# MaxWolf-01/sentinel2-landcover-classification

Measured on AMD Instinct MI355X. Metric: Sentinel-2 256x256x13 tiles/sec fwd+bwd, higher is better.
Workload: dtype f32

## Files before the change

__graft_entry__.py:

```python
from __future__ import annotations

import os
import subprocess
import sys
from pathlib import Path

ROOT = Path(__file__).resolve().parent
PKG = ROOT / "sentinel2-landcover-classification_amd"
CSRC = PKG / "csrc"
LIB = PKG / "libs2k.so"
SOURCES = ["s2k_api.hip", "igemm.hip", "igemm_pc.hip", "conv_dma.hip", "conv_q4.hip", "conv_bf16.hip", "wgrad.hip", "wgrad_pc.hip", "wgrad_q4.hip", "wgrad_bf16.hip", "dwconv.hip", "ew.hip", "loss.hip", "vit.hip", "attn.hip", "input.hip", "predict.hip", "flat_stats.hip", "quicklook.hip", "peaks.hip"]


def _stale() -> bool:
    if not LIB.exists():
        return True
    t = LIB.stat().st_mtime
    deps = [CSRC / s for s in SOURCES] + [CSRC / "common.h", CSRC / "wgrad.h", CSRC / "igemm.h", CSRC / "dma.h", ROOT / "include" / "s2k.h", ROOT / "include" / "s2k_ops.h"]
    return any(d.stat().st_mtime > t for d in deps)


def build_tuning(stamps: bool = False, exact_silu: bool = False) -> Path:
    hipcc = os.environ.get("HIPCC", "/opt/rocm/bin/hipcc")
    out = PKG / ("libs2k_exact.so" if exact_silu else ("libs2k_stamps.so" if stamps else "libs2k_tuning.so"))
    cmd = ([hipcc, "--offload-arch=gfx950", "-O3", "-std=c++17", "-fPIC", "-Wno-unused-value", "-DS2K_TUNING"] + (["-DS2K_DMA_STAMPS"] if stamps else [])
           + (["-DS2K_EXACT_SILU"] if exact_silu else []) + ["-shared", "-o", str(out)])
    cmd += [str(CSRC / s) for s in SOURCES]
    r = subprocess.run(cmd, stdout=subprocess.PIPE, stderr=subprocess.STDOUT, text=True)
    if r.returncode != 0:
        raise RuntimeError(f"tuning build failed:\n{r.stdout}")
    return out


def build(force: bool = False) -> None:
    if str(ROOT) not in sys.path:
        sys.path.insert(0, str(ROOT))
    hipcc = os.environ.get("HIPCC", "/opt/rocm/bin/hipcc")
    have_hipcc = Path(hipcc).exists()
    if (force or _stale()) and have_hipcc:
        objs = []
        procs = []
        for s in SOURCES:
            obj = CSRC / (s + ".o")
            objs.append(str(obj))
# ... 104 lines not shown
```

include/s2k_ops.h:

```cpp
#ifndef S2K_OPS_H
#define S2K_OPS_H

#define S2K_N_T 12
#define S2K_N_N 4
#define S2K_N_D 24
#define S2K_N_F 6

#define S2K_BASE_WS 0
#define S2K_BASE_PARAMS 1
#define S2K_BASE_GRADS 2
#define S2K_BASE_BUFS 3
#define S2K_BASE_X 4
#define S2K_BASE_OUT 5
#define S2K_BASE_DOUT 6
#define S2K_BASE_NOISE 7
#define S2K_BASE_WGS 8
#define S2K_BASE_CONST 9
#define S2K_BASE_Y 10
#define S2K_BASE_AUX 11
#define S2K_BASE_WPACK 12
#define S2K_BASE_DX 13
#define S2K_N_BASES 14

#define S2K_PRO_NONE 0
#define S2K_PRO_AFFINE 1
#define S2K_PRO_SILU 2
#define S2K_PRO_RELU 3
#define S2K_PRO_GELU 4
#define S2K_MODE_CONV 0
#define S2K_MODE_CONVT_SCATTER 1
#define S2K_MODE_GATHER2X2 2
#define S2K_FLAG_SIDE 1
#define S2K_FLAG_JOIN 2
#define S2K_FLAG_BF16 4
#define S2K_FLAG_Q4 16
#define S2K_FLAG_DMA 8
#define S2K_FLAG_RES_GELU_GRAD 32
#define S2K_FLAG_SPLIT 64
#define S2K_FLAG_CHAIN 128

#define S2K_OP_MEMSET 1
#define S2K_MEMSET_T_DST 0
#define S2K_MEMSET_N_BYTES 0

#define S2K_OP_AXPY 2
#define S2K_AXPY_T_X 0
#define S2K_AXPY_T_Y 1
#define S2K_AXPY_N_COUNT 0

#define S2K_OP_WEIGHT_PACK 3
#define S2K_WEIGHT_PACK_T_TABLE 0
#define S2K_WEIGHT_PACK_T_SRC 1
#define S2K_WEIGHT_PACK_T_DST 2
#define S2K_WEIGHT_PACK_N_TOTAL 0
#define S2K_WEIGHT_PACK_N_BF16_BASE 1
#define S2K_WEIGHT_PACK_N_Q4_BASE 2
#define S2K_WEIGHT_PACK_N_SPLIT_BASE 3
#define S2K_WEIGHT_PACK_D_N_ENTRIES 0

#define S2K_OP_CONV 4
#define S2K_CONV_T_X1 0
#define S2K_CONV_T_BNV1 1
#define S2K_CONV_T_GATE1 2
#define S2K_CONV_T_X2 3
#define S2K_CONV_T_BNV2 4
#define S2K_CONV_T_WT 5
#define S2K_CONV_T_BIAS 6
#define S2K_CONV_T_Y 7
#define S2K_CONV_T_STATS 8
#define S2K_CONV_T_RES 9
#define S2K_CONV_T_SCRATCH 10
#define S2K_CONV_T_WTB 11
// ... 722 lines not shown
```

sentinel2-landcover-classification_amd/csrc/s2k_api.hip:

```cpp
#include <cstdarg>
#include <cstdio>
#include <cstring>
#include <mutex>
#include <vector>

#include <stdlib.h>

#include "common.h"

namespace s2k {

static thread_local char g_err[512] = "";
thread_local int g_s2k_variant = 0;

void set_error(const char* fmt, ...) {
    va_list ap;
    va_start(ap, fmt);
    vsnprintf(g_err, sizeof(g_err), fmt, ap);
    va_end(ap);
}

int launch_conv(const S2kOp&, const Ctx&);
int launch_wgrad(const S2kOp&, const Ctx&);
int launch_dwconv_fwd(const S2kOp&, const Ctx&);
int launch_dwconv_dgrad(const S2kOp&, const Ctx&);
int launch_dwconv_wgrad(const S2kOp&, const Ctx&);
int launch_axpy(const S2kOp&, const Ctx&);
int launch_weight_pack(const S2kOp&, const Ctx&);
int launch_wgrad_finalize(const S2kOp&, const Ctx&);
int launch_bn_finalize(const S2kOp&, const Ctx&);
int launch_se_pool(const S2kOp&, const Ctx&);
int launch_se_fc(const S2kOp&, const Ctx&);
// ... 11 lines not shown
int launch_chan_ln_bwd(const S2kOp&, const Ctx&);
int launch_act_bwd(const S2kOp&, const Ctx&);
int launch_act_fwd(const S2kOp&, const Ctx&);
int launch_attn_fwd(const S2kOp&, const Ctx&);
int launch_attn_bwd(const S2kOp&, const Ctx&);
int launch_mae_mask_index(const S2kOp&, const Ctx&);
int launch_token_gather(const S2kOp&, const Ctx&);
int launch_token_scatter(const S2kOp&, const Ctx&);
int launch_patchify(const S2kOp&, const Ctx&);
int launch_mae_loss_fwd(const S2kOp&, const Ctx&);
int launch_mae_loss_bwd(const S2kOp&, const Ctx&);
int launch_transpose_cl(const S2kOp&, const Ctx&);
int launch_drop_gate(const S2kOp&, const Ctx&);
int launch_confusion(const S2kOp&, const Ctx&);
int launch_tile_prep(const S2kOp&, const Ctx&);
int launch_se_bn_sums(const S2kOp&, const Ctx&);
int launch_se_bn_combine(const S2kOp&, const Ctx&);
int launch_space_to_depth(const S2kOp&, const Ctx&);
int launch_se_fc_wgrad(const S2kOp&, const Ctx&);
int launch_ids_to_dec_idx(const S2kOp&, const Ctx&);
int launch_upsample_zero(const S2kOp&, const Ctx&);
int launch_im2col(const S2kOp&, const Ctx&);
int launch_tile_label_hist(const S2kOp&, const Ctx&);
int launch_tile_moments(const S2kOp&, const Ctx&);
int launch_window_blend(const S2kOp&, const Ctx&);
int launch_seg_stats(const S2kOp&, const Ctx&);
int launch_seg_hist(const S2kOp&, const Ctx&);
int launch_grad_clip(const S2kOp&, const Ctx&);
int launch_tile_radix_hist(const S2kOp&, const Ctx&);
int launch_tile_rank_pick(const S2kOp&, const Ctx&);
int launch_tile_quicklook(const S2kOp&, const Ctx&);
int launch_class_overlay(const S2kOp&, const Ctx&);
int launch_dw_bwd_chain(const S2kOp*, const Ctx&);
int launch_adam(float*, const float*, float*, float*, int64_t, double, double, double, double, double, int, hipStream_t);
int launch_mfma_selftest(const float*, const float*, float*, hipStream_t);

static int launch_memset(const S2kOp& op, const Ctx& c) {
    const int64_t ref = op.t[S2K_MEMSET_T_DST];
    const int64_t bytes = op.n[S2K_MEMSET_N_BYTES];
    if (ref < 0 || bytes <= 0) { set_error("memset: bad args"); return S2K_EINVAL; }
    const int base = (int)(ref >> 56);
    if (base >= c.n_bases || !c.bases[base]) { set_error("memset: null base %d", base); return S2K_EFAULT; }
    char* dst = static_cast<char*>(c.bases[base]) + (ref & ((1ll << 56) - 1));
    if (hipMemsetAsync(dst, 0, (size_t)bytes, c.stream) != hipSuccess) { set_error("memset: hipMemsetAsync failed"); return S2K_EHIP; }
    return S2K_OK;
}

static const char* const kNames[S2K_N_KINDS + 1] = {
    nullptr,
    "MEMSET", "AXPY", "WEIGHT_PACK", "CONV", "WGRAD", "WGRAD_FINALIZE", "DWCONV_FWD", "DWCONV_DGRAD", "DWCONV_WGRAD",
    "BN_FINALIZE", "SE_POOL", "SE_FC", "SE_FC_BWD", "SE_BWD_REDUCE", "BN_BWD_REDUCE", "BN_BWD_FINALIZE", "BN_BWD_APPLY",
    "BN_RESIDUAL", "CHANNEL_SUM", "LOSS_FWD", "LOSS_BWD", "ARGMAX", "CHAN_LN_FWD", "CHAN_LN_BWD", "ACT_BWD", "ACT_FWD",
    "ATTN_FWD", "ATTN_BWD", "MAE_MASK_INDEX", "IDS_TO_DEC_IDX", "TOKEN_GATHER", "TOKEN_SCATTER", "PATCHIFY", "MAE_LOSS_FWD",
    "MAE_LOSS_BWD", "TRANSPOSE_CL", "CONFUSION", "DROP_GATE", "TILE_PREP", "SE_BN_SUMS", "SE_BN_COMBINE", "SPACE_TO_DEPTH",
    "UPSAMPLE_ZERO", "SE_FC_WGRAD", "IM2COL", "TILE_LABEL_HIST", "TILE_MOMENTS", "WINDOW_BLEND",
    "SEG_STATS", "SEG_HIST", "GRAD_CLIP", "TILE_RADIX_HIST", "TILE_RANK_PICK", "TILE_QUICKLOOK", "CLASS_OVERLAY"};

static int dispatch(const S2kOp& op, const Ctx& c) {
    switch (op.kind) {
        case S2K_OP_MEMSET: return launch_memset(op, c);
        case S2K_OP_AXPY: return launch_axpy(op, c);
        case S2K_OP_WEIGHT_PACK: return launch_weight_pack(op, c);
        case S2K_OP_CONV: return launch_conv(op, c);
        case S2K_OP_WGRAD: return launch_wgrad(op, c);
        case S2K_OP_WGRAD_FINALIZE: return launch_wgrad_finalize(op, c);
        case S2K_OP_DWCONV_FWD: return launch_dwconv_fwd(op, c);
// ... 141 lines not shown
};

static int try_dw_chain(const S2kOp* ops, int i, int end, const Ctx& c, int* rc) {
    if (!(ops[i].flags & S2K_FLAG_CHAIN) || i + 3 >= end) return 0;
    const S2kOp &a1 = ops[i], &wg = ops[i + 1], &dg = ops[i + 2], &a2 = ops[i + 3];
    if (a1.kind != S2K_OP_BN_BWD_APPLY || wg.kind != S2K_OP_DWCONV_WGRAD || dg.kind != S2K_OP_DWCONV_DGRAD || a2.kind != S2K_OP_BN_BWD_APPLY) return 0;
    if ((a1.flags | wg.flags | dg.flags | a2.flags) & (S2K_FLAG_BF16 | S2K_FLAG_SPLIT)) return 0;
    const int64_t dy = a1.t[S2K_BN_BWD_APPLY_T_DY], x = dg.t[S2K_DWCONV_DGRAD_T_XRAW], g = dg.t[S2K_DWCONV_DGRAD_T_G];
    if (dy < 0 || a1.t[S2K_BN_BWD_APPLY_T_GP] != dy || a1.t[S2K_BN_BWD_APPLY_T_COEF] >= 0 || a1.t[S2K_BN_BWD_APPLY_T_PS] < 0 ||
        a1.t[S2K_BN_BWD_APPLY_T_MULBC] < 0 || a1.t[S2K_BN_BWD_APPLY_T_ADDBC] < 0 || a1.d[S2K_BN_BWD_APPLY_D_ACT] != S2K_PRO_SILU ||
        a1.d[S2K_BN_BWD_APPLY_D_EVAL] || a1.d[S2K_BN_BWD_APPLY_D_OUT_BF16] || a1.n[S2K_BN_BWD_APPLY_N_COUNT] <= 0) return 0;
    if (wg.t[S2K_DWCONV_WGRAD_T_DY] != dy || dg.t[S2K_DWCONV_DGRAD_T_DY] != dy || x < 0 || wg.t[S2K_DWCONV_WGRAD_T_X] != x ||
        dg.t[S2K_DWCONV_DGRAD_T_BNV] < 0 || wg.t[S2K_DWCONV_WGRAD_T_BNV] != dg.t[S2K_DWCONV_DGRAD_T_BNV] || g < 0 || g == dy || g == x ||
        dg.t[S2K_DWCONV_DGRAD_T_STATS2] < 0) return 0;
    for (int k = 0; k <= 10; ++k)
        if (wg.d[k] != dg.d[k]) return 0;
    const int B = dg.d[0], C = dg.d[1], H = dg.d[2], W = dg.d[3], K = dg.d[4];
    if (B <= 0 || C <= 0 || H != W || (W != 8 && W != 16) || (K != 3 && K != 5) || dg.d[5] != 1 || dg.d[6] != (K - 1) / 2 || dg.d[7] != (K - 1) / 2 ||
        dg.d[8] != H || dg.d[9] != W || dg.d[10] != S2K_PRO_SILU || dg.d[S2K_DWCONV_DGRAD_D_BETA] != 0) return 0;
    if ((int64_t)B * C * H * W * 4 >= 0x7ffffff0ll) return 0;
    if (a2.t[S2K_BN_BWD_APPLY_T_GP] != g || a2.t[S2K_BN_BWD_APPLY_T_DY] != g || a2.t[S2K_BN_BWD_APPLY_T_Y] != x ||
        a2.t[S2K_BN_BWD_APPLY_T_BNV] != dg.t[S2K_DWCONV_DGRAD_T_BNV] || a2.t[S2K_BN_BWD_APPLY_T_STATS2] != dg.t[S2K_DWCONV_DGRAD_T_STATS2] ||
        a2.t[S2K_BN_BWD_APPLY_T_COEF] >= 0 || a2.t[S2K_BN_BWD_APPLY_T_PS] >= 0 || a2.t[S2K_BN_BWD_APPLY_T_MULBC] >= 0 ||
        a2.t[S2K_BN_BWD_APPLY_T_ADDBC] >= 0 || a2.d[S2K_BN_BWD_APPLY_D_ACT] != S2K_PRO_NONE || a2.d[S2K_BN_BWD_APPLY_D_EVAL] ||
        a2.d[S2K_BN_BWD_APPLY_D_OUT_BF16] || a2.n[S2K_BN_BWD_APPLY_N_COUNT] <= 0) return 0;
    const int HW = H * W;
    if (a1.d[S2K_BN_BWD_APPLY_D_B] != B || a1.d[S2K_BN_BWD_APPLY_D_C] != C || a1.d[S2K_BN_BWD_APPLY_D_HW] != HW ||
        a2.d[S2K_BN_BWD_APPLY_D_B] != B || a2.d[S2K_BN_BWD_APPLY_D_C] != C || a2.d[S2K_BN_BWD_APPLY_D_HW] != HW) return 0;
    g_s2k_variant = 0;
    *rc = check_launch(launch_dw_bwd_chain(&ops[i], c), ops[i], i);
    return 4;
}

int s2k_program_run(const S2kOp* ops, int begin, int end, void* const* bases, int n_bases, void* stream) {
    if (!ops || !bases || begin < 0 || end < begin) { set_error("program_run: bad arguments"); return S2K_EINVAL; }
    hipStream_t main_st = static_cast<hipStream_t>(stream);
    DeviceGuard guard(main_st);
    Ctx c{bases, n_bases, main_st};
    bool any_side = false;
    for (int i = begin; i < end && !any_side; ++i) any_side = (ops[i].flags & S2K_FLAG_SIDE) != 0;
    SideQueue* sq = any_side ? lease_side_queue(guard.dev) : nullptr;
    bool side_busy = false;
    bool main_dirty = true;
    auto join = [&]() {
        if (!side_busy) return;
        (void)hipEventRecord(sq->join, sq->stream);
        (void)hipStreamWaitEvent(main_st, sq->join, 0);
        side_busy = false;
    };
    int rc = S2K_OK;
    for (int i = begin; i < end; ++i) {
        const S2kOp& op = ops[i];
        if ((op.flags & S2K_FLAG_CHAIN) && i + 3 < end) {
            if ((op.flags | ops[i + 1].flags | ops[i + 2].flags | ops[i + 3].flags) & S2K_FLAG_JOIN) join();
            const int used = try_dw_chain(ops, i, end, c, &rc);
            if (used) {
                main_dirty = true;
                if (rc != S2K_OK) break;
                i += used - 1;
                continue;
            }
        }
        if ((op.flags & S2K_FLAG_SIDE) && sq) {
            if (main_dirty) {
                (void)hipEventRecord(sq->fork, main_st);
                (void)hipStreamWaitEvent(sq->stream, sq->fork, 0);
                main_dirty = false;
            }
            Ctx cs{bases, n_bases, sq->stream};
            rc = check_launch(dispatch(op, cs), op, i);
            side_busy = true;
        } else {
            if (op.flags & S2K_FLAG_JOIN) join();
            rc = check_launch(dispatch(op, c), op, i);
            main_dirty = true;
        }
        if (rc != S2K_OK) break;
    }
    join();
    release_side_queue(guard.dev, sq);
    return rc;
}

int s2k_op_launch(const S2kOp* op, void* const* bases, int n_bases, void* stream) {
    if (!op || !bases) { set_error("op_launch: bad arguments"); return S2K_EINVAL; }
    DeviceGuard guard(static_cast<hipStream_t>(stream));
    Ctx c{bases, n_bases, static_cast<hipStream_t>(stream)};
    return check_launch(dispatch(*op, c), *op, 0);
}

static int profile_impl(const S2kOp* ops, int begin, int end, void* const* bases, int n_bases, void* stream, float* ms_by_kind,
                        int* launches_by_kind, float* ms_per_op, int* variant_per_op);

int s2k_program_profile(const S2kOp* ops, int begin, int end, void* const* bases, int n_bases, void* stream, float* ms_by_kind,
                        int* launches_by_kind) {
// ... 3 lines not shown
int s2k_program_profile_ops(const S2kOp* ops, int begin, int end, void* const* bases, int n_bases, void* stream,
                            float* ms_per_op) {
    float ms[S2K_N_KINDS + 1];
    int cnt[S2K_N_KINDS + 1];
    return profile_impl(ops, begin, end, bases, n_bases, stream, ms, cnt, ms_per_op, nullptr);
}

int s2k_program_profile_variants(const S2kOp* ops, int begin, int end, void* const* bases, int n_bases, void* stream,
                                 float* ms_per_op, int* variant_per_op) {
    float ms[S2K_N_KINDS + 1];
    int cnt[S2K_N_KINDS + 1];
    if (!ms_per_op || !variant_per_op) { set_error("program_profile_variants: bad arguments"); return S2K_EINVAL; }
    return profile_impl(ops, begin, end, bases, n_bases, stream, ms, cnt, ms_per_op, variant_per_op);
}

static int profile_impl(const S2kOp* ops, int begin, int end, void* const* bases, int n_bases, void* stream, float* ms_by_kind,
                        int* launches_by_kind, float* ms_per_op, int* variant_per_op) {
    if (!ops || !bases || !ms_by_kind || !launches_by_kind || begin < 0 || end < begin) {
        set_error("program_profile: bad arguments");
        return S2K_EINVAL;
    }
    hipStream_t st = static_cast<hipStream_t>(stream);
    DeviceGuard guard(st);
    Ctx c{bases, n_bases, st};
    const int n = end - begin;
    hipEvent_t* ev = new hipEvent_t[n + 1];
    for (int i = 0; i <= n; ++i) hipEventCreate(&ev[i]);
    int rc = S2K_OK;
    hipEventRecord(ev[0], st);
    int done = 0;
    std::vector<char> fused(n, 0);
    for (int i = 0; i < n; ++i) {
        g_s2k_variant = 0;
        const int used = try_dw_chain(ops, begin + i, end, c, &rc);
        if (!used) rc = check_launch(dispatch(ops[begin + i], c), ops[begin + i], begin + i);
        if (rc != S2K_OK) break;
        for (int k = 0; k < (used ? used : 1); ++k) {
            if (variant_per_op) variant_per_op[i + k] = g_s2k_variant;
            hipEventRecord(ev[i + k + 1], st);
            if (k) fused[i + k] = 1;
        }
        if (used) i += used - 1;
        done = i + 1;
    }
    hipStreamSynchronize(st);
    if (rc == S2K_OK) {
        for (int k = 0; k <= S2K_N_KINDS; ++k) { ms_by_kind[k] = 0.0f; launches_by_kind[k] = 0; }
        for (int i = 0; i < done; ++i) {
            float ms = 0.0f;
            if (!fused[i]) hipEventElapsedTime(&ms, ev[i], ev[i + 1]);
            const int k = ops[begin + i].kind;
            if (ms_per_op) ms_per_op[i] = ms;
            if (k > 0 && k <= S2K_N_KINDS && !fused[i]) { ms_by_kind[k] += ms; launches_by_kind[k] += 1; }
        }
    }
    for (int i = 0; i <= n; ++i) hipEventDestroy(ev[i]);
    delete[] ev;
    return rc;
}

int s2k_adam_step(float* p, const float* g, float* m, float* v, int64_t n, double lr, double beta1, double beta2, double eps,
                  double weight_decay, int step, void* stream) {
    DeviceGuard guard(static_cast<hipStream_t>(stream));
    const int rc = launch_adam(p, g, m, v, n, lr, beta1, beta2, eps, weight_decay, step, static_cast<hipStream_t>(stream));
    if (rc != S2K_OK) return rc;
    const hipError_t e = hipGetLastError();
// ... 15 lines not shown
```

sentinel2-landcover-classification_amd/plan/opdefs.py:

```python
from __future__ import annotations

N_T, N_N, N_D, N_F = 12, 4, 24, 6
OP_BYTES = 8 + 8 * N_T + 8 * N_N + 4 * N_D + 4 * N_F
assert OP_BYTES == 256

BASES = ["WS", "PARAMS", "GRADS", "BUFS", "X", "OUT", "DOUT", "NOISE", "WGS", "CONST", "Y", "AUX", "WPACK", "DX"]
BASE = {n: i for i, n in enumerate(BASES)}

def stats_replicas(C: int) -> int:
    return max(1, min(64, 4096 // max(C, 1)))


PRO_NONE, PRO_AFFINE, PRO_SILU, PRO_RELU, PRO_GELU = 0, 1, 2, 3, 4
ACT_NONE, ACT_SILU, ACT_RELU, ACT_GELU = 0, 2, 3, 4
ACT_MUL = 5
MODE_CONV, MODE_CONVT_SCATTER, MODE_GATHER2X2 = 0, 1, 2
FLAG_SIDE, FLAG_JOIN = 1, 2
FLAG_BF16 = 4
FLAG_Q4 = 16
FLAG_RES_GELU_GRAD = 32
FLAG_SPLIT = 64
FLAG_DMA = 8
FLAG_CHAIN = 128

FOLD_T, FOLD_N, FOLD_D, FOLD_F = ["FSTATS", "FGAMMA", "FBETA", "FRM", "FRV"], ["FCOUNT"], ["FNREP"], ["FEPS", "FMOM"]
FOLD_KINDS = ("DWCONV_FWD", "SE_POOL", "BN_RESIDUAL")

OPS: dict[str, tuple[list[str], list[str], list[str], list[str]]] = {
    "MEMSET": (["DST"], ["BYTES"], [], []),
    "AXPY": (["X", "Y"], ["COUNT"], [], []),
    "WEIGHT_PACK": (["TABLE", "SRC", "DST"], ["TOTAL", "BF16_BASE", "Q4_BASE", "SPLIT_BASE"], ["N_ENTRIES"], []),
    "CONV": (["X1", "BNV1", "GATE1", "X2", "BNV2", "WT", "BIAS", "Y", "STATS", "RES", "SCRATCH", "WTB"], [],
             ["B", "C1", "C2", "H", "W", "M", "KH", "KW", "STRIDE", "PAD_T", "PAD_L", "HO", "WO",
              "PRO1", "PRO2", "MODE", "W_SM", "W_SK", "W_ST", "FLIP", "BETA", "YC", "NREP", "X1_BF16"], []),
    "WGRAD": (["P", "BNVP", "GATEP", "Q", "BNVQ", "GATEQ", "WGS"], [],
              ["B", "M", "C", "CTOT", "H", "W", "KH", "KW", "STRIDE", "PAD_T", "PAD_L", "HO", "WO",
               "PROP", "PROQ", "MODE", "P_BF16"], []),
    "WGRAD_FINALIZE": (["TABLE", "WGS", "GRADS"], ["TOTAL"], ["N_ENTRIES"], []),
    "DWCONV_FWD": (["X", "BNV", "WT", "Y", "STATS"] + FOLD_T, FOLD_N,
                   ["B", "C", "H", "W", "K", "STRIDE", "PAD_T", "PAD_L", "HO", "WO", "PRO", "NREP"] + FOLD_D, FOLD_F),
    "DWCONV_DGRAD": (["DY", "WT", "XRAW", "BNV", "G", "STATS2"], [],
                     ["B", "C", "H", "W", "K", "STRIDE", "PAD_T", "PAD_L", "HO", "WO", "PRO", "BETA", "NREP"], []),
    "DWCONV_WGRAD": (["DY", "X", "BNV", "DW"], [],
                     ["B", "C", "H", "W", "K", "STRIDE", "PAD_T", "PAD_L", "HO", "WO", "PRO"], []),
    "BN_FINALIZE": (["STATS", "GAMMA", "BETA", "RM", "RV", "BNV"], ["COUNT"], ["C", "TRAIN", "NREP"], ["EPS", "MOM"]),
    "SE_POOL": (["Y", "BNV", "POOL"] + FOLD_T, FOLD_N, ["B", "C", "HW", "PRO"] + FOLD_D, FOLD_F),
    "SE_FC": (["POOL", "W1", "B1", "W2", "B2", "HPRE", "GATE"], [], ["B", "C", "CSQ"], []),
    "SE_FC_BWD": (["DGATE", "GATE", "HPRE", "POOL", "W1", "W2", "DW1", "DB1", "DW2", "DB2", "DPOOL", "HS"], [],
                  ["B", "C", "CSQ"], []),
    "SE_BWD_REDUCE": (["G", "Y", "BNV", "DGATE"], [], ["B", "C", "HW", "PRO"], []),
    "BN_BWD_REDUCE": (["G", "Y", "BNV", "MULBC", "ADDBC", "NOISE", "GOUT", "STATS2"], [],
                      ["B", "C", "HW", "ACT", "NREP"], ["KEEP", "ADDSCALE"]),
    "BN_BWD_FINALIZE": (["STATS2", "GAMMA", "BNV", "DGAMMA", "DBETA", "COEF"], ["COUNT"], ["C", "NREP"], []),
    "BN_BWD_APPLY": (["GP", "Y", "BNV", "COEF", "DY", "STATS2", "GAMMA", "DGAMMA", "DBETA", "MULBC", "ADDBC", "PS"], ["COUNT"],
                     ["B", "C", "HW", "NREP", "ACT", "EVAL", "OUT_BF16"], ["ADDSCALE"]),
    "BN_RESIDUAL": (["Y", "BNV", "IDENT", "NOISE", "XOUT"] + FOLD_T, FOLD_N, ["B", "C", "HW"] + FOLD_D, ["KEEP"] + FOLD_F),
# ... 85 lines not shown
```

sentinel2-landcover-classification_amd/plan/unet_plan.py:

```python
from __future__ import annotations

import math
from dataclasses import dataclass, field

from . import opdefs as D
from .program import Arena, Program, TRef

CAT_SIZES = {
    "b0": [592, 296, 152, 80], "b1": [592, 296, 152, 80], "b2": [600, 304, 152, 80],
    "b3": [608, 304, 160, 88], "b4": [624, 312, 160, 88], "b5": [640, 320, 168, 88],
    "b6": [656, 328, 168, 96], "b7": [672, 336, 176, 96],
}


@dataclass
class BlockSpec:
    kernel: int
    stride: int
    cin: int
    cout: int
    expand: int
    se: int
    residual: bool

# ... 717 lines not shown
        if bwd_aux_end > fwd_aux_end:
            pre_ops.append(("MEMSET", dict(DST=TRef(D.BASE["AUX"], fwd_aux_end, (1,), "f32"),
                                           BYTES=bwd_aux_end - fwd_aux_end)))
        p.bwd.ops[0:0] = pre_ops
        segments = _bucket_backward(p, layout, table, bucket_floats)
        side_max = float(tune("S2K_SIDE_MAX_GFLOP", "1e9")) * 1e9
        finalize_on_side = tune("S2K_FINALIZE_SIDE", "1") != "0"
        for kind, f in p.bwd.ops:
            if kind == "WGRAD" and 2.0 * f["M"] * f["C"] * f["KH"] * f["KW"] * f["B"] * f["HO"] * f["WO"] > side_max:
                continue
            if kind in ("WGRAD", "DWCONV_WGRAD", "CHANNEL_SUM", "SE_FC_WGRAD"):
                f["_flags"] = D.FLAG_SIDE
            elif kind == "WGRAD_FINALIZE":
                f["_flags"] = D.FLAG_SIDE if finalize_on_side else D.FLAG_JOIN
        side_stream_hazards(p.bwd)
        n_before = len(p.bwd.ops)
        attach_q4()
        if not bwd_pack_in_fwd:
            pack_op(p.bwd, p.pack_rows["bwd"])
        if len(p.bwd.ops) > n_before:
            segments = [(a + 1 if a else 0, b + 1, lo, hi) for (a, b, lo, hi) in segments]
        bwd = p.bwd
    else:
        attach_q4()
    pack_op(p.fwd, p.pack_rows["fwd"])
    if bwd_pack_in_fwd:
        pack_op(p.fwd, p.pack_rows["bwd"], D.FLAG_SIDE)
    attach_splitk_scratch()
    if getattr(p, "bf16", False):
        mark_bf16(p, bwd)
    if getattr(p, "split", False):
        mark_split(p, bwd)
    mark_dw_chain(p, bwd, segments)
    return segments, bwd


def side_stream_hazards(prog: Program) -> int:
    def ranges(f, names):
        out = []
        for k in names:
            v = f.get(k)
            if isinstance(v, TRef):
                out.append((v.base, v.off, v.off + v.nbytes))
        return out

    pending: list = []
    added = 0
    for kind, f in prog.ops:
        flags = f.get("_flags", 0)
        t_names = D.OPS[kind][0]
        writes = D.WRITES.get(kind, tuple(t_names))
        if flags & D.FLAG_SIDE:
            pending.extend(ranges(f, [k for k in t_names if k not in writes]))
            continue
        if flags & D.FLAG_JOIN:
            pending.clear()
            continue
        if pending:
            for (b, lo, hi) in ranges(f, writes):
                if any(b == pb and lo < phi and plo < hi for (pb, plo, phi) in pending):
                    f["_flags"] = flags | D.FLAG_JOIN
                    pending.clear()
                    added += 1
                    break
    return added

# ... 92 lines not shown
        if tuple(k for k, _ in ops[i:i + 4]) != kinds or seg_end.get(i, 0) < i + 4:
            continue
        a1, wg, dg, a2 = (f for _, f in ops[i:i + 4])
        if any(f.get("_flags", 0) & bad_flags for f in (a1, wg, dg, a2)):
            continue
        dy, x, g, st2 = a1.get("DY"), dg.get("XRAW"), dg.get("G"), dg.get("STATS2")
        if not (same(a1.get("GP"), dy) and same(wg.get("DY"), dy) and same(dg.get("DY"), dy)
                and same(wg.get("X"), x) and same(a2.get("Y"), x) and same(a2.get("GP"), g) and same(a2.get("DY"), g)
                and same(a2.get("STATS2"), st2) and same(wg.get("BNV"), dg.get("BNV")) and same(a2.get("BNV"), dg.get("BNV"))):
            continue
        if not (a1.get("ACT") == D.ACT_SILU and isinstance(a1.get("PS"), TRef) and isinstance(a1.get("MULBC"), TRef)
                and isinstance(a1.get("ADDBC"), TRef) and a1.get("COEF") is None and not a1.get("EVAL") and not a1.get("OUT_BF16")):
            continue
        if not (a2.get("COEF") is None and not a2.get("ACT") and a2.get("PS") is None and a2.get("MULBC") is None
                and a2.get("ADDBC") is None and not a2.get("EVAL") and not a2.get("OUT_BF16")):
            continue
        geo = ("B", "C", "H", "W", "K", "STRIDE", "PAD_T", "PAD_L", "HO", "WO", "PRO")
        K, W = dg["K"], dg["W"]
        if not (all(wg[k] == dg[k] for k in geo) and dg["STRIDE"] == 1 and dg["PRO"] == D.PRO_SILU and not dg.get("BETA")
                and dg["H"] == W and W in (8, 16) and K in (3, 5) and dg["HO"] == W and dg["WO"] == W
                and dg["PAD_T"] == (K - 1) // 2 and dg["PAD_L"] == (K - 1) // 2):
            continue
        if not all(f["B"] == dg["B"] and f["C"] == dg["C"] and f["HW"] == W * W for f in (a1, a2)):
            continue
        dead = [(t.base, t.off, t.off + t.nbytes) for t in (st2,)]
        live = False
        for _k2, f2 in ops[i + 4:]:
            for v in f2.values():
                if isinstance(v, TRef) and any(v.base == b and v.off < hi and lo < v.off + v.nbytes for (b, lo, hi) in dead):
                    live = True
        if live:
            continue
        a1["_flags"] = a1.get("_flags", 0) | D.FLAG_CHAIN
        marked += 1
    return marked


def fold_bn_finalize(prog: Program) -> int:
    if tune("S2K_FOLD_BN", "1") != "1":
        return 0
    ops = prog.ops
    folded = 0
    i = 0
    while i < len(ops):
        kind, f = ops[i]
        if kind != "BN_FINALIZE" or not f.get("TRAIN") or f.get("_flags"):
            i += 1
            continue
        bnv = f["BNV"]
        touched = {t.ref for k in ("BNV", "RM", "RV", "STATS") if isinstance(t := f.get(k), TRef)}
        target = None
        for j in range(i + 1, len(ops)):
            k2, f2 = ops[j]
            refs = {v.ref for v in f2.values() if isinstance(v, TRef)}
            if not (refs & touched):
                continue
            if (k2 in D.FOLD_KINDS and isinstance(f2.get("BNV"), TRef) and f2["BNV"].ref == bnv.ref and f2.get("FSTATS") is None
                    and f2.get("C") == f["C"] and f2.get("PRO", 1) and len(refs & touched) == 1 and not f2.get("_flags")):
                target = j
            break
        if target is None:
            i += 1
            continue
        ops[target][1].update(FSTATS=f["STATS"], FGAMMA=f["GAMMA"], FBETA=f["BETA"], FRM=f["RM"], FRV=f["RV"], FCOUNT=f["COUNT"],
                              FNREP=f["NREP"], FEPS=f["EPS"], FMOM=f["MOM"])
        del ops[i]
# ... 107 lines not shown
```

Before: 999.9.

## Fuse BN backward reduce and apply into paired kernels without materialized gradient

Adds a bn_pair path that detects adjacent BN_BWD_REDUCE/BN_BWD_APPLY ops writing the pre-BN gradient in place. It recomputes that gradient (mul/add/drop-connect/activation grad) inside both the reduce and apply kernels instead of writing it out and reading it back. For small spatial sizes a single per-channel kernel does the reduction and the apply, optionally keeping the loaded data in registers. The aim is to cut memory traffic and one launch per BN backward, at the cost of recomputing the activation gradient and adding planner and runtime matching logic.

Result: no change. 1007 (median of 6 runs) (+0.7%).

```diff
diff --git a/__graft_entry__.py b/__graft_entry__.py
--- a/__graft_entry__.py
+++ b/__graft_entry__.py
@@ -9,7 +9,7 @@
 PKG = ROOT / "sentinel2-landcover-classification_amd"
 CSRC = PKG / "csrc"
 LIB = PKG / "libs2k.so"
-SOURCES = ["s2k_api.hip", "igemm.hip", "igemm_pc.hip", "conv_dma.hip", "conv_q4.hip", "conv_bf16.hip", "wgrad.hip", "wgrad_pc.hip", "wgrad_q4.hip", "wgrad_bf16.hip", "dwconv.hip", "ew.hip", "loss.hip", "vit.hip", "attn.hip", "input.hip", "predict.hip", "flat_stats.hip", "quicklook.hip", "peaks.hip"]
+SOURCES = ["s2k_api.hip", "igemm.hip", "igemm_pc.hip", "conv_dma.hip", "conv_q4.hip", "conv_bf16.hip", "wgrad.hip", "wgrad_pc.hip", "wgrad_q4.hip", "wgrad_bf16.hip", "dwconv.hip", "ew.hip", "bn_pair.hip", "loss.hip", "vit.hip", "attn.hip", "input.hip", "predict.hip", "flat_stats.hip", "quicklook.hip", "peaks.hip"]
 
 
 def _stale() -> bool:
diff --git a/include/s2k_ops.h b/include/s2k_ops.h
--- a/include/s2k_ops.h
+++ b/include/s2k_ops.h
@@ -38,6 +38,7 @@
 #define S2K_FLAG_RES_GELU_GRAD 32
 #define S2K_FLAG_SPLIT 64
 #define S2K_FLAG_CHAIN 128
+#define S2K_FLAG_BN_PAIR 256
 
 #define S2K_OP_MEMSET 1
 #define S2K_MEMSET_T_DST 0
diff --git a/sentinel2-landcover-classification_amd/csrc/bn_pair.hip b/sentinel2-landcover-classification_amd/csrc/bn_pair.hip
--- /dev/null
+++ b/sentinel2-landcover-classification_amd/csrc/bn_pair.hip
@@ -0,0 +1,309 @@
+#include "common.h"
+
+namespace s2k {
+
+namespace {
+
+constexpr int PAIR_CHUNK = 4096;
+constexpr int PAIR_SMALL_HW = 256;
+constexpr int PAIR_SMALL_C = 512;
+
+template <typename T>
+T* ref_ptr(const Ctx& c, int64_t ref) {
+    if (ref < 0) return nullptr;
+    const int base = (int)(ref >> 56);
+    const int64_t off = ref & ((1ll << 56) - 1);
+    if (base >= c.n_bases || c.bases[base] == nullptr) return reinterpret_cast<T*>(1);
+    return reinterpret_cast<T*>(static_cast<char*>(c.bases[base]) + off);
+}
+bool bad(const void* q) { return q == reinterpret_cast<const void*>(1); }
+
+struct PairTask {
+    int64_t plane;
+    int start, count;
+};
+
+__device__ __forceinline__ bool pair_task(int HW, int64_t nplanes, PairTask& t) {
+    const int chunks = (HW + PAIR_CHUNK - 1) / PAIR_CHUNK;
+    const int64_t task = (int64_t)blockIdx.x * 4 + (threadIdx.x >> 6);
+    if (task >= nplanes * chunks) return false;
+    t.plane = (int64_t)((uint32_t)task / (uint32_t)chunks);
+    const int ck = (int)(task - t.plane * chunks);
+    t.start = ck * PAIR_CHUNK;
+    t.count = min(PAIR_CHUNK, HW - t.start);
+    return true;
+}
+
+struct PairArgs {
+    const float *g, *y, *bnv, *mulbc, *addbc, *noise;
+    int C, HW, act;
+    int64_t nplanes;
+    float keep, addscale;
+};
+
+__device__ __forceinline__ void pair_mul_add(const PairArgs& p, int64_t plane, int b, float& mul, float& add) {
+    mul = p.mulbc ? p.mulbc[plane] : 1.0f;
+    if (p.noise) mul *= floorf(p.keep + p.noise[b]) / p.keep;
+    add = p.addbc ? p.addbc[plane] * p.addscale : 0.0f;
+}
+
+__device__ __forceinline__ float pair_gp(float g, float y, float mul, float add, float scale, float shift, int act) {
+    float v = fmaf(g, mul, add);
+    if (act != S2K_PRO_NONE) v *= act_grad(fmaf(y, scale, shift), act);
+    return v;
+}
+
+}
+
+template <bool VEC>
+__global__ void __launch_bounds__(NTHREADS) bn_pair_reduce_kernel(const PairArgs p, double* stats2, int nrep) {
+    PairTask t;
+    if (!pair_task(p.HW, p.nplanes, t)) return;
+    const int lane = threadIdx.x & 63;
+    const int C = p.C;
+    const int c = (int)((uint32_t)t.plane % (uint32_t)C);
+    const int b = (int)((uint32_t)t.plane / (uint32_t)C);
+    const float scale = p.bnv[c], shift = p.bnv[C + c], mean = p.bnv[2 * C + c], invstd = p.bnv[3 * C + c];
+    float mul, add;
+    pair_mul_add(p, t.plane, b, mul, add);
+    const int64_t base = t.plane * p.HW + t.start;
+    const float* g = p.g + base;
+    const float* y = p.y + base;
+    float s1 = 0.0f, s2 = 0.0f;
+    if (VEC) {
+        const int n4 = t.count >> 2;
+        for (int i = lane; i < n4; i += 128) {
+            const int j = min(i + 64, n4 - 1);
+            const bool second = i + 64 < n4;
+            const float4 g0 = reinterpret_cast<const float4*>(g)[i], y0 = reinterpret_cast<const float4*>(y)[i];
+            const float4 g1 = reinterpret_cast<const float4*>(g)[j], y1 = reinterpret_cast<const float4*>(y)[j];
+            const float* gp0 = &g0.x;
+            const float* yp0 = &y0.x;
+            const float* gp1 = &g1.x;
+            const float* yp1 = &y1.x;
+#pragma unroll
+            for (int k = 0; k < 4; ++k) {
+                const float v = pair_gp(gp0[k], yp0[k], mul, add, scale, shift, p.act);
+                s1 += v;
+                s2 = fmaf(v, (yp0[k] - mean) * invstd, s2);
+            }
+#pragma unroll
+            for (int k = 0; k < 4; ++k) {
+                float v = pair_gp(gp1[k], yp1[k], mul, add, scale, shift, p.act);
+                v = second ? v : 0.0f;
+                s1 += v;
+                s2 = fmaf(v, (yp1[k] - mean) * invstd, s2);
+            }
+        }
+    } else {
+        for (int i = lane; i < t.count; i += 64) {
+            const float yy = y[i];
+            const float v = pair_gp(g[i], yy, mul, add, scale, shift, p.act);
+            s1 += v;
+            s2 = fmaf(v, (yy - mean) * invstd, s2);
+        }
+    }
+    s1 = wave_sum(s1);
+    s2 = wave_sum(s2);
+    if (lane == 0) {
+        double* st = stats2 + (int64_t)(blockIdx.x % nrep) * 2 * C;
+        atomic_add_d(st + c, (double)s1);
+        atomic_add_d(st + C + c, (double)s2);
+    }
+}
+
+template <bool VEC>
+__global__ void __launch_bounds__(NTHREADS) bn_pair_apply_kernel(const PairArgs p, float* out, const BnFuse fz) {
+    PairTask t;
+    if (!pair_task(p.HW, p.nplanes, t)) return;
+    const int lane = threadIdx.x & 63;
+    const int C = p.C;
+    const int c = (int)((uint32_t)t.plane % (uint32_t)C);
+    const int b = (int)((uint32_t)t.plane / (uint32_t)C);
+    const int64_t base = t.plane * p.HW + t.start;
+    const float* g = p.g + base;
+    const float* y = p.y + base;
+    float* o = out + base;
+    const int n4 = t.count >> 2;
+    float4 gv0 = make_float4(0, 0, 0, 0), yv0 = make_float4(0, 0, 0, 0);
+    if (VEC && lane < n4) {
+        gv0 = reinterpret_cast<const float4*>(g)[lane];
+        yv0 = reinterpret_cast<const float4*>(y)[lane];
+    }
+    const float scale = p.bnv[c], shift = p.bnv[C + c], mean = p.bnv[2 * C + c], invstd = p.bnv[3 * C + c];
+    float mul, add;
+    pair_mul_add(p, t.plane, b, mul, add);
+    double s1, s2;
+    bn_fuse_sums(fz, C, c, lane, s1, s2);
+    const double aa = (double)fz.gamma[c] * (double)invstd;
+    const float A = (float)aa, Bq = (float)(-aa * s2 * fz.inv_count), Cq = (float)(-aa * s1 * fz.inv_count);
+    const float k0 = A, k1 = Bq * invstd, k2 = Cq - Bq * invstd * mean;
+    if (t.plane < C && t.start == 0 && lane == 0) {
+        fz.dgamma[c] += (float)s2;
+        fz.dbeta[c] += (float)s1;
+    }
+    if (VEC) {
+        for (int i = lane; i < n4; i += 64) {
+            const float4 gv = gv0, yv = yv0;
+            if (i + 64 < n4) {
+                gv0 = reinterpret_cast<const float4*>(g)[i + 64];
+                yv0 = reinterpret_cast<const float4*>(y)[i + 64];
+            }
+            float4 r;
+            r.x = fmaf(k0, pair_gp(gv.x, yv.x, mul, add, scale, shift, p.act), fmaf(k1, yv.x, k2));
+            r.y = fmaf(k0, pair_gp(gv.y, yv.y, mul, add, scale, shift, p.act), fmaf(k1, yv.y, k2));
+            r.z = fmaf(k0, pair_gp(gv.z, yv.z, mul, add, scale, shift, p.act), fmaf(k1, yv.z, k2));
+            r.w = fmaf(k0, pair_gp(gv.w, yv.w, mul, add, scale, shift, p.act), fmaf(k1, yv.w, k2));
+            reinterpret_cast<float4*>(o)[i] = r;
+        }
+    } else {
+        for (int i = lane; i < t.count; i += 64) {
+            const float yy = y[i];
+            o[i] = fmaf(k0, pair_gp(g[i], yy, mul, add, scale, shift, p.act), fmaf(k1, yy, k2));
+        }
+    }
+}
+
+template <int U, bool KEEP>
+__global__ void __launch_bounds__(NTHREADS) bn_pair_small_kernel(const PairArgs p, float* out, const BnFuse fz, int B) {
+    __shared__ double red[8];
+    const int c = blockIdx.x, C = p.C, HW = p.HW;
+    const int n4 = HW >> 2, items = B * n4;
+    const float scale = p.bnv[c], shift = p.bnv[C + c], mean = p.bnv[2 * C + c], invstd = p.bnv[3 * C + c];
+    float4 gv[U], yv[U];
+    float mul[U], add[U];
+    int64_t off[U];
+    double d1 = 0.0, d2 = 0.0;
+    auto load = [&](int q0) {
+#pragma unroll
+        for (int u = 0; u < U; ++u) {
+            const int q = min(q0 + u * NTHREADS, items - 1);
+            const int b = (int)((uint32_t)q / (uint32_t)n4), li = q - b * n4;
+            const int64_t plane = (int64_t)b * C + c;
+            off[u] = plane * HW + 4 * li;
+            gv[u] = *reinterpret_cast<const float4*>(p.g + off[u]);
+            yv[u] = *reinterpret_cast<const float4*>(p.y + off[u]);
+            pair_mul_add(p, plane, b, mul[u], add[u]);
+        }
+    };
+    const int lane = threadIdx.x & 63;
+    const bool aligned = (n4 & (n4 - 1)) == 0;
+    for (int w0 = threadIdx.x - lane; w0 < items; w0 += U * NTHREADS) {
+        const int q0 = w0 + lane;
+        load(q0);
+        float t1 = 0.0f, t2 = 0.0f;
+#pragma unroll
+        for (int u = 0; u < U; ++u) {
+            const bool ok = q0 + u * NTHREADS < items;
+            const float* gp = &gv[u].x;
+            const float* yp = &yv[u].x;
+            float s1 = 0.0f, s2 = 0.0f;
+#pragma unroll
+            for (int k = 0; k < 4; ++k) {
+                const float v = pair_gp(gp[k], yp[k], mul[u], add[u], scale, shift, p.act);
+                s1 += v;
+                s2 = fmaf(v, (yp[k] - mean) * invstd, s2);
+            }
+            s1 = ok ? s1 : 0.0f;
+            s2 = ok ? s2 : 0.0f;
+            if (aligned) {
+                s1 = group_sum(s1, n4);
+                s2 = group_sum(s2, n4);
+                const bool first = (q0 & (n4 - 1)) == 0;
+                d1 += first ? (double)s1 : 0.0;
+                d2 += first ? (double)s2 : 0.0;
+            } else {
+                t1 += s1;
+                t2 += s2;
+            }
+        }
+        d1 += (double)t1;
+        d2 += (double)t2;
+    }
+    d1 = wave_sum_d(d1);
+    d2 = wave_sum_d(d2);
+    if ((threadIdx.x & 63) == 0) { red[threadIdx.x >> 6] = d1; red[4 + (threadIdx.x >> 6)] = d2; }
+    __syncthreads();
+    const double s1 = ((red[0] + red[1]) + red[2]) + red[3], s2 = ((red[4] + red[5]) + red[6]) + red[7];
+    const double aa = (double)fz.gamma[c] * (double)invstd;
+    const float A = (float)aa, Bq = (float)(-aa * s2 * fz.inv_count), Cq = (float)(-aa * s1 * fz.inv_count);
+    const float k0 = A, k1 = Bq * invstd, k2 = Cq - Bq * invstd * mean;
+    if (threadIdx.x == 0) {
+        fz.dgamma[c] += (float)s2;
+        fz.dbeta[c] += (float)s1;
+    }
+    for (int q0 = threadIdx.x; q0 < items; q0 += U * NTHREADS) {
+        if (!KEEP) load(q0);
+#pragma unroll
+        for (int u = 0; u < U; ++u) {
+            if (q0 + u * NTHREADS >= items) break;
+            const float4 g = gv[u], y = yv[u];
+            float4 r;
+            r.x = fmaf(k0, pair_gp(g.x, y.x, mul[u], add[u], scale, shift, p.act), fmaf(k1, y.x, k2));
+            r.y = fmaf(k0, pair_gp(g.y, y.y, mul[u], add[u], scale, shift, p.act), fmaf(k1, y.y, k2));
+            r.z = fmaf(k0, pair_gp(g.z, y.z, mul[u], add[u], scale, shift, p.act), fmaf(k1, y.z, k2));
+            r.w = fmaf(k0, pair_gp(g.w, y.w, mul[u], add[u], scale, shift, p.act), fmaf(k1, y.w, k2));
+            *reinterpret_cast<float4*>(out + off[u]) = r;
+        }
+    }
+}
+
+int launch_bn_pair(const S2kOp* o, const Ctx& c, hipEvent_t mid, int* took) {
+    *took = 0;
+    const S2kOp &r = o[0], &a = o[1];
+    PairArgs p{};
+    p.g = ref_ptr<const float>(c, r.t[S2K_BN_BWD_REDUCE_T_G]);
+    p.y = ref_ptr<const float>(c, r.t[S2K_BN_BWD_REDUCE_T_Y]);
+    p.bnv = ref_ptr<const float>(c, r.t[S2K_BN_BWD_REDUCE_T_BNV]);
+    p.mulbc = ref_ptr<const float>(c, r.t[S2K_BN_BWD_REDUCE_T_MULBC]);
+    p.addbc = ref_ptr<const float>(c, r.t[S2K_BN_BWD_REDUCE_T_ADDBC]);
+    p.noise = ref_ptr<const float>(c, r.t[S2K_BN_BWD_REDUCE_T_NOISE]);
+    float* out = ref_ptr<float>(c, a.t[S2K_BN_BWD_APPLY_T_DY]);
+    double* st2 = ref_ptr<double>(c, r.t[S2K_BN_BWD_REDUCE_T_STATS2]);
+    BnFuse fz{};
+    fz.st2 = st2;
+    fz.gamma = ref_ptr<const float>(c, a.t[S2K_BN_BWD_APPLY_T_GAMMA]);
+    fz.dgamma = ref_ptr<float>(c, a.t[S2K_BN_BWD_APPLY_T_DGAMMA]);
+    fz.dbeta = ref_ptr<float>(c, a.t[S2K_BN_BWD_APPLY_T_DBETA]);
+    const void* ptrs[] = {p.g, p.y, p.bnv, p.mulbc, p.addbc, p.noise, out, st2, fz.gamma, fz.dgamma, fz.dbeta};
+    for (const void* q : ptrs)
+        if (bad(q)) { set_error("bn_pair: tensor references a null base"); return S2K_EFAULT; }
+    const int B = r.d[S2K_BN_BWD_REDUCE_D_B], C = r.d[S2K_BN_BWD_REDUCE_D_C], HW = r.d[S2K_BN_BWD_REDUCE_D_HW];
+    const int64_t count = a.n[S2K_BN_BWD_APPLY_N_COUNT];
+    if (!p.g || !p.y || !p.bnv || !out || !st2 || !fz.gamma || !fz.dgamma || !fz.dbeta || B <= 0 || C <= 0 || HW <= 0 || count <= 0) return S2K_OK;
+    const int64_t nplanes = (int64_t)B * C;
+    const int64_t tasks = nplanes * ((HW + PAIR_CHUNK - 1) / PAIR_CHUNK);
+    if (nplanes * HW * 4 >= 0x7ffffff0ll || tasks >= 0xffffffffll) return S2K_OK;
+    p.C = C; p.HW = HW; p.nplanes = nplanes;
+    p.act = r.d[S2K_BN_BWD_REDUCE_D_ACT];
+    p.keep = r.f[S2K_BN_BWD_REDUCE_F_KEEP];
+    p.addscale = r.f[S2K_BN_BWD_REDUCE_F_ADDSCALE];
+    fz.inv_count = 1.0 / (double)count;
+    fz.nrep = r.d[S2K_BN_BWD_REDUCE_D_NREP] > 0 ? r.d[S2K_BN_BWD_REDUCE_D_NREP] : 1;
+    const int64_t items = (int64_t)B * (HW >> 2);
+    if (HW <= PAIR_SMALL_HW && (HW & 3) == 0 && (items <= 2 * NTHREADS || C >= PAIR_SMALL_C)) {
+        if (items <= 2 * NTHREADS)
+            hipLaunchKernelGGL((bn_pair_small_kernel<2, true>), dim3(C), dim3(NTHREADS), 0, c.stream, p, out, fz, B);
+        else if (items <= 8 * NTHREADS)
+            hipLaunchKernelGGL((bn_pair_small_kernel<8, true>), dim3(C), dim3(NTHREADS), 0, c.stream, p, out, fz, B);
+        else
+            hipLaunchKernelGGL((bn_pair_small_kernel<4, false>), dim3(C), dim3(NTHREADS), 0, c.stream, p, out, fz, B);
+        *took = 2;
+        return S2K_OK;
+    }
+    if (HW <= 64 && (HW & 3) == 0 && B >= 2) return S2K_OK;
+    const unsigned blocks = (unsigned)cdiv64(tasks, 4);
+    if ((HW & 3) == 0) {
+        hipLaunchKernelGGL((bn_pair_reduce_kernel<true>), dim3(blocks), dim3(NTHREADS), 0, c.stream, p, st2, fz.nrep);
+        if (mid) (void)hipEventRecord(mid, c.stream);
+        hipLaunchKernelGGL((bn_pair_apply_kernel<true>), dim3(blocks), dim3(NTHREADS), 0, c.stream, p, out, fz);
+    } else {
+        hipLaunchKernelGGL((bn_pair_reduce_kernel<false>), dim3(blocks), dim3(NTHREADS), 0, c.stream, p, st2, fz.nrep);
+        if (mid) (void)hipEventRecord(mid, c.stream);
+        hipLaunchKernelGGL((bn_pair_apply_kernel<false>), dim3(blocks), dim3(NTHREADS), 0, c.stream, p, out, fz);
+    }
+    *took = 1;
+    return S2K_OK;
+}
+
+}
diff --git a/sentinel2-landcover-classification_amd/csrc/s2k_api.hip b/sentinel2-landcover-classification_amd/csrc/s2k_api.hip
--- a/sentinel2-landcover-classification_amd/csrc/s2k_api.hip
+++ b/sentinel2-landcover-classification_amd/csrc/s2k_api.hip
@@ -1,3 +1,4 @@
+#include <algorithm>
 #include <cstdarg>
 #include <cstdio>
 #include <cstring>
@@ -75,6 +76,7 @@
 int launch_tile_quicklook(const S2kOp&, const Ctx&);
 int launch_class_overlay(const S2kOp&, const Ctx&);
 int launch_dw_bwd_chain(const S2kOp*, const Ctx&);
+int launch_bn_pair(const S2kOp*, const Ctx&, hipEvent_t, int*);
 int launch_adam(float*, const float*, float*, float*, int64_t, double, double, double, double, double, int, hipStream_t);
 int launch_mfma_selftest(const float*, const float*, float*, hipStream_t);
 
@@ -282,6 +284,30 @@
     return 4;
 }
 
+static int try_bn_pair(const S2kOp* ops, int i, int end, const Ctx& c, int* rc, hipEvent_t mid = nullptr) {
+    if (!(ops[i].flags & S2K_FLAG_BN_PAIR) || i + 1 >= end) return 0;
+    const S2kOp &r = ops[i], &a = ops[i + 1];
+    if (r.kind != S2K_OP_BN_BWD_REDUCE || a.kind != S2K_OP_BN_BWD_APPLY) return 0;
+    if ((r.flags | a.flags) & (S2K_FLAG_BF16 | S2K_FLAG_SPLIT | S2K_FLAG_SIDE)) return 0;
+    const int64_t gout = r.t[S2K_BN_BWD_REDUCE_T_GOUT], st2 = r.t[S2K_BN_BWD_REDUCE_T_STATS2];
+    if (gout < 0 || st2 < 0 || a.t[S2K_BN_BWD_APPLY_T_GP] != gout || a.t[S2K_BN_BWD_APPLY_T_DY] != gout ||
+        r.t[S2K_BN_BWD_REDUCE_T_Y] < 0 || r.t[S2K_BN_BWD_REDUCE_T_Y] == gout || a.t[S2K_BN_BWD_APPLY_T_Y] != r.t[S2K_BN_BWD_REDUCE_T_Y] ||
+        r.t[S2K_BN_BWD_REDUCE_T_BNV] < 0 || a.t[S2K_BN_BWD_APPLY_T_BNV] != r.t[S2K_BN_BWD_REDUCE_T_BNV] || a.t[S2K_BN_BWD_APPLY_T_STATS2] != st2) return 0;
+    if (a.d[S2K_BN_BWD_APPLY_D_B] != r.d[S2K_BN_BWD_REDUCE_D_B] || a.d[S2K_BN_BWD_APPLY_D_C] != r.d[S2K_BN_BWD_REDUCE_D_C] ||
+        a.d[S2K_BN_BWD_APPLY_D_HW] != r.d[S2K_BN_BWD_REDUCE_D_HW] ||
+        std::max(a.d[S2K_BN_BWD_APPLY_D_NREP], 1) != std::max(r.d[S2K_BN_BWD_REDUCE_D_NREP], 1)) return 0;
+    if (a.t[S2K_BN_BWD_APPLY_T_COEF] >= 0 || a.t[S2K_BN_BWD_APPLY_T_PS] >= 0 || a.t[S2K_BN_BWD_APPLY_T_MULBC] >= 0 ||
+        a.t[S2K_BN_BWD_APPLY_T_ADDBC] >= 0 || a.d[S2K_BN_BWD_APPLY_D_ACT] != S2K_PRO_NONE || a.d[S2K_BN_BWD_APPLY_D_EVAL] ||
+        a.d[S2K_BN_BWD_APPLY_D_OUT_BF16] || a.n[S2K_BN_BWD_APPLY_N_COUNT] <= 0 || a.t[S2K_BN_BWD_APPLY_T_GAMMA] < 0 ||
+        a.t[S2K_BN_BWD_APPLY_T_DGAMMA] < 0 || a.t[S2K_BN_BWD_APPLY_T_DBETA] < 0) return 0;
+    int took = 0;
+    const int st = launch_bn_pair(&ops[i], c, mid, &took);
+    if (st == S2K_OK && !took) return 0;
+    *rc = check_launch(st, ops[i], i);
+    g_s2k_variant = took == 2 ? 17 : 16;
+    return 2;
+}
+
 int s2k_program_run(const S2kOp* ops, int begin, int end, void* const* bases, int n_bases, void* stream) {
     if (!ops || !bases || begin < 0 || end < begin) { set_error("program_run: bad arguments"); return S2K_EINVAL; }
     hipStream_t main_st = static_cast<hipStream_t>(stream);
@@ -311,6 +337,16 @@
                 continue;
             }
         }
+        if ((op.flags & S2K_FLAG_BN_PAIR) && i + 1 < end) {
+            if ((op.flags | ops[i + 1].flags) & S2K_FLAG_JOIN) join();
+            const int used = try_bn_pair(ops, i, end, c, &rc);
+            if (used) {
+                main_dirty = true;
+                if (rc != S2K_OK) break;
+                i += used - 1;
+                continue;
+            }
+        }
         if ((op.flags & S2K_FLAG_SIDE) && sq) {
             if (main_dirty) {
                 (void)hipEventRecord(sq->fork, main_st);
@@ -380,6 +416,18 @@
     std::vector<char> fused(n, 0);
     for (int i = 0; i < n; ++i) {
         g_s2k_variant = 0;
+        if (i + 1 < n && try_bn_pair(ops, begin + i, end, c, &rc, ev[i + 1])) {
+            if (rc != S2K_OK) break;
+            if (variant_per_op) variant_per_op[i] = variant_per_op[i + 1] = g_s2k_variant;
+            if (g_s2k_variant == 17) {
+                hipEventRecord(ev[i + 1], st);
+                fused[i + 1] = 1;
+            }
+            hipEventRecord(ev[i + 2], st);
+            i += 1;
+            done = i + 1;
+            continue;
+        }
         const int used = try_dw_chain(ops, begin + i, end, c, &rc);
         if (!used) rc = check_launch(dispatch(ops[begin + i], c), ops[begin + i], begin + i);
         if (rc != S2K_OK) break;
diff --git a/sentinel2-landcover-classification_amd/plan/opdefs.py b/sentinel2-landcover-classification_amd/plan/opdefs.py
--- a/sentinel2-landcover-classification_amd/plan/opdefs.py
+++ b/sentinel2-landcover-classification_amd/plan/opdefs.py
@@ -22,6 +22,8 @@
 FLAG_SPLIT = 64
 FLAG_DMA = 8
 FLAG_CHAIN = 128
+FLAG_BN_PAIR = 256
+BN_PAIR_SMALL_HW = 256
 
 FOLD_T, FOLD_N, FOLD_D, FOLD_F = ["FSTATS", "FGAMMA", "FBETA", "FRM", "FRV"], ["FCOUNT"], ["FNREP"], ["FEPS", "FMOM"]
 FOLD_KINDS = ("DWCONV_FWD", "SE_POOL", "BN_RESIDUAL")
diff --git a/sentinel2-landcover-classification_amd/plan/unet_plan.py b/sentinel2-landcover-classification_amd/plan/unet_plan.py
--- a/sentinel2-landcover-classification_amd/plan/unet_plan.py
+++ b/sentinel2-landcover-classification_amd/plan/unet_plan.py
@@ -773,6 +773,7 @@
     if getattr(p, "split", False):
         mark_split(p, bwd)
     mark_dw_chain(p, bwd, segments)
+    mark_bn_pairs(p, bwd, segments)
     return segments, bwd
 
 
@@ -931,6 +932,46 @@
         if live:
             continue
         a1["_flags"] = a1.get("_flags", 0) | D.FLAG_CHAIN
+        marked += 1
+    return marked
+
+
+def mark_bn_pairs(p: "_P", bwd, segments=None) -> int:
+    if bwd is None or tune("S2K_BN_PAIR", "1") != "1":
+        return 0
+    ops = bwd.ops
+    seg_end = {}
+    for (a, b, _lo, _hi) in (segments or [(0, len(ops), 0, 0)]):
+        for i in range(a, b):
+            seg_end[i] = b
+    bad_flags = D.FLAG_BF16 | D.FLAG_SPLIT | D.FLAG_SIDE
+
+    def same(a, b):
+        return isinstance(a, TRef) and isinstance(b, TRef) and a.ref == b.ref
+
+    marked = 0
+    for i in range(len(ops) - 1):
+        (k0, r), (k1, a) = ops[i], ops[i + 1]
+        if (k0, k1) != ("BN_BWD_REDUCE", "BN_BWD_APPLY") or seg_end.get(i, 0) < i + 2:
+            continue
+        if (r.get("_flags", 0) | a.get("_flags", 0)) & bad_flags:
+            continue
+        gout = r.get("GOUT")
+        if not (same(a.get("GP"), gout) and same(a.get("DY"), gout) and same(a.get("Y"), r.get("Y")) and not same(r.get("Y"), gout)
+                and same(a.get("BNV"), r.get("BNV")) and same(a.get("STATS2"), r.get("STATS2"))):
+            continue
+        if not (all(a[k] == r[k] for k in ("B", "C", "HW")) and max(a.get("NREP", 0), 1) == max(r.get("NREP", 0), 1)):
+            continue
+        if not (a.get("COEF") is None and a.get("PS") is None and a.get("MULBC") is None and a.get("ADDBC") is None and not a.get("ACT")
+                and not a.get("EVAL") and not a.get("OUT_BF16") and a.get("COUNT", 0) > 0
+                and all(isinstance(a.get(k), TRef) for k in ("GAMMA", "DGAMMA", "DBETA"))):
+            continue
+        if r["HW"] <= D.BN_PAIR_SMALL_HW and r["HW"] % 4 == 0:
+            st2 = r["STATS2"]
+            if any(isinstance(v, TRef) and v.base == st2.base and v.off < st2.off + st2.nbytes and st2.off < v.off + v.nbytes
+                   for _k2, f2 in ops[i + 2:] for v in f2.values()):
+                continue
+        r["_flags"] = r.get("_flags", 0) | D.FLAG_BN_PAIR
         marked += 1
     return marked
 
```
